# miuda-ai/lele

Measured on AMD Instinct MI355X. Metric: STFT+mel GB/s (SenseVoice front-end: PCM -> log-mel -> LFR, algorithmic bytes); SenseVoiceSmall-shaped RTF in `sensevoice`, higher is better.
Workload: dtype f32

## Files before the change

### lele_amd/csrc/frontend.hip

```cpp
#include <type_traits>
#include "common.h"
#include "fe_core.h"

#include <math.h>

#include <algorithm>

using namespace lele;

namespace {

constexpr int kMaxMelRounds = 8;

struct FeDev {
    const float* tw_re;
    const float* tw_im;
    const float2* tw;
    const float* window;
    const float* melw;
    const int* mel_start;
    const int* mel_step_off;
    int mel_rounds;
    int mel_steps;
    int n_mels;
    int lfr_m, lfr_n;
};

struct GridBlock {
    __device__ __forceinline__ unsigned x() const { return blockIdx.x; }
    __device__ __forceinline__ unsigned y() const { return blockIdx.y; }
};
struct SegBlock {
    unsigned bx;
    __device__ __forceinline__ unsigned x() const { return bx; }
    __device__ __forceinline__ unsigned y() const { return 0u; }
};

struct FeSeg {
    int64_t start, len;
    int64_t num_frames, t_lfr;
    int64_t row0;
    int64_t block0;
};

constexpr int kSumRows = 66;
constexpr int kSumPitch = 164;

__global__ __launch_bounds__(64) void fe_frame_sum_kernel(const float* __restrict__ pcm, int64_t utt_stride,
                                                          int64_t pcm_len, int64_t num_frames,
                                                          float* __restrict__ mean_out, int aligned16) {
    __shared__ __attribute__((aligned(16))) float tile[kSumRows * kSumPitch];
    const int lane = threadIdx.x;
    const int64_t f0 = (int64_t)blockIdx.x * 64;
    const float* base = pcm + (int64_t)blockIdx.y * utt_stride;
    const int64_t s0 = f0 * fe::kHop;
    constexpr int kVecPerRow = fe::kHop / 4;
    constexpr int kVecs = kSumRows * kVecPerRow;
    constexpr int kIters = (kVecs + 63) / 64;
    constexpr int kBatch = 14;
    static_assert(kIters % kBatch == 0, "batching");
    for (int b0 = 0; b0 < kIters; b0 += kBatch) {
        float4 st[kBatch];
#pragma unroll
        for (int u = 0; u < kBatch; ++u) {
            const int idx = (b0 + u) * 64 + lane;
            int64_t s = s0 + 4 * (int64_t)idx;
            if (s + 3 >= pcm_len) s = aligned16 ? ((pcm_len - 4) & ~int64_t(3)) : (pcm_len - 4);
            if (s < 0) s = 0;
            const float* src = base + s;
            if (aligned16) {
                st[u] = *reinterpret_cast<const float4*>(src);
            } else {
                st[u] = make_float4(src[0], src[1], src[2], src[3]);
            }
        }
#pragma unroll
        for (int u = 0; u < kBatch; ++u) {
            const int idx = (b0 + u) * 64 + lane;
            if (idx < kVecs) {
                float4 xv = st[u];
                xv.x *= 32768.0f;
                xv.y *= 32768.0f;
                xv.z *= 32768.0f;
                xv.w *= 32768.0f;
                const int row = idx / kVecPerRow, c = idx - row * kVecPerRow;
                *reinterpret_cast<float4*>(&tile[row * kSumPitch + 4 * c]) = xv;
            }
        }
    }
    __syncthreads();
    float sum = 0.0f;
#pragma unroll
    for (int seg = 0; seg < 3; ++seg) {
        const float* rowp = &tile[(lane + seg) * kSumPitch];
        const int nvec = seg < 2 ? kVecPerRow : (fe::kFrame - 2 * fe::kHop) / 4;
#pragma unroll 10
        for (int k = 0; k < nvec; ++k) {
            const float4 r = *reinterpret_cast<const float4*>(rowp + 4 * k);
            sum = sum + r.x;
            sum = sum + r.y;
            sum = sum + r.z;
            sum = sum + r.w;
        }
    }
    const int64_t f = f0 + lane;
    if (f < num_frames) mean_out[(int64_t)blockIdx.y * num_frames + f] = sum / (float)fe::kFrame;
}

constexpr int kFrameXchgFloats = 2 * 16 * fe::kXchgPitch;
constexpr int kWaveLdsFloats = 4 * kFrameXchgFloats;
constexpr int kPStride = 272;

struct TwLds {
    const float2* t;
    __device__ __forceinline__ float2 at(int i) const { return t[i]; }
};

template <int MODE>
__device__ __forceinline__ float lane_rot_prev(float v, int p) {
    if (MODE == 1) {
        return __builtin_bit_cast(float,
                                  __builtin_amdgcn_update_dpp(0, __builtin_bit_cast(int, v), 0x121, 0xf, 0xf, true));
    } else {
        return __shfl(v, (p + 15) & 15, 16);
    }
}

constexpr int kStdMelLen[5] = {3, 4, 6, 10, 17};
constexpr int kStdMelOff[6] = {0, 3, 7, 13, 23, 40};

template <int MODE, bool STDMEL, bool FUSED, int PASSES, bool LOWREG, class Blk>
__device__ __forceinline__ void fe_main_body(const float* __restrict__ pcm, int64_t utt_stride,
                                             int64_t num_frames, int64_t t_lfr,
                                             const float* __restrict__ means, const FeDev& tb,
                                             float* __restrict__ out, float* __restrict__ logmel_out,
                                             int aligned16, float* s_melw, Blk bl) {
    constexpr int FR = 16 * PASSES;
    constexpr int kRows = FR + 2;
    constexpr int kXFloats = FUSED ? (kRows * kSumPitch > 4 * kWaveLdsFloats ? kRows * kSumPitch : 4 * kWaveLdsFloats)
                                   : 4 * kWaveLdsFloats;
    __shared__ float2 s_tw[LOWREG ? 480 : 512];
    __shared__ __attribute__((aligned(16))) float s_x[kXFloats];
    __shared__ float s_mean[64];
    __shared__ int s_mstart[16 * (STDMEL ? 5 : kMaxMelRounds)];
    __shared__ int s_moff[kMaxMelRounds + 1];
    constexpr int kTwBase = LOWREG ? 31 : 0;

    for (int i = threadIdx.x; i < 511 - kTwBase; i += 256) s_tw[i] = tb.tw[i + kTwBase];
    if (!STDMEL)
        for (int i = threadIdx.x; i < tb.mel_steps * 16; i += 256) s_melw[i] = tb.melw[i];
    if (threadIdx.x < tb.mel_rounds * 16) s_mstart[threadIdx.x] = tb.mel_start[threadIdx.x];
    if (threadIdx.x <= tb.mel_rounds) s_moff[threadIdx.x] = tb.mel_step_off[threadIdx.x];
    const int lane = threadIdx.x & 63, wave = threadIdx.x >> 6;
    const int g = lane >> 4, p = lane & 15;
    if (FUSED) {
        const float* ubase = pcm + (int64_t)bl.y() * utt_stride;
        const int64_t s0 = (int64_t)bl.x() * FR * fe::kHop;
        constexpr int kVecPerRow = fe::kHop / 4;
        constexpr int kVecs = kRows * kVecPerRow;
        constexpr int kIters = (kVecs + 255) / 256;
        float4 st[kIters];
#pragma unroll
        for (int u = 0; u < kIters; ++u) {
            const int idx = u * 256 + (int)threadIdx.x;
            int64_t sidx = s0 + 4 * (int64_t)idx;
            if (sidx + 3 >= utt_stride) sidx = aligned16 ? ((utt_stride - 4) & ~int64_t(3)) : (utt_stride - 4);
            if (sidx < 0) sidx = 0;
            const float* src = ubase + sidx;
            if (aligned16)
                st[u] = *reinterpret_cast<const float4*>(src);
            else
                st[u] = make_float4(src[0], src[1], src[2], src[3]);
        }
#pragma unroll
        for (int u = 0; u < kIters; ++u) {
            const int idx = u * 256 + (int)threadIdx.x;
            if (idx < kVecs) {
                float4 xv = st[u];
                xv.x *= 32768.0f;
                xv.y *= 32768.0f;
                xv.z *= 32768.0f;
                xv.w *= 32768.0f;
                const int row = idx / kVecPerRow, c = idx - row * kVecPerRow;
                *reinterpret_cast<float4*>(&s_x[row * kSumPitch + 4 * c]) = xv;
            }
        }
        __syncthreads();
    }
    const int h = fe::rev4(p);
    float* xw = s_x + wave * kWaveLdsFloats;
    float* xf = xw + g * kFrameXchgFloats;
    const float* base = pcm + (int64_t)bl.y() * utt_stride;
    const float* mean_u = means + (int64_t)bl.y() * num_frames;
    const int d_out = tb.n_mels * tb.lfr_m;
    float* out_u = out ? out + (int64_t)bl.y() * t_lfr * d_out : nullptr;
    float* lm_u = logmel_out ? logmel_out + (int64_t)bl.y() * num_frames * tb.n_mels : nullptr;

    float win[fe::kQ];
    if (!LOWREG) {
#pragma unroll
        for (int q = 0; q < fe::kQ; ++q) win[q] = tb.window[p + 16 * q];
    }

    float xr[fe::kQ];
    float mean_next = 0.0f;
    auto issue_loads = [&](int pass) {
        const int64_t f = (int64_t)bl.x() * FR + wave * (4 * PASSES) + pass * 4 + g;
        const int64_t fc = f < num_frames ? f : 0;
        const float* src = base + fc * fe::kHop + p;
        if (!FUSED) mean_next = mean_u[fc];
#pragma unroll
        for (int q = 0; q < fe::kQ; ++q) xr[q] = src[16 * q];
    };
    issue_loads(0);
    if (FUSED) {
        constexpr int kVecPerRow = fe::kHop / 4;
        if (wave == 0 && lane < FR) {
            float sum = 0.0f;
#pragma unroll
            for (int seg = 0; seg < 3; ++seg) {
                const float* rowp = &s_x[(lane + seg) * kSumPitch];
                const int nvec = seg < 2 ? kVecPerRow : (fe::kFrame - 2 * fe::kHop) / 4;
#pragma unroll 10
                for (int k = 0; k < nvec; ++k) {
                    const float4 r = *reinterpret_cast<const float4*>(rowp + 4 * k);
                    sum = sum + r.x;
                    sum = sum + r.y;
                    sum = sum + r.z;
                    sum = sum + r.w;
                }
            }
            s_mean[lane] = sum / (float)fe::kFrame;
        }
    }
    __syncthreads();

    auto run_pass = [&](int pass, auto load_next_c) {
        constexpr bool load_next = decltype(load_next_c)::value;
        const int64_t f = (int64_t)bl.x() * FR + wave * (4 * PASSES) + pass * 4 + g;
        const bool valid = f < num_frames;
        const float mean = FUSED ? s_mean[wave * (4 * PASSES) + pass * 4 + g] : mean_next;
        if (LOWREG) {
            int off = 0;
            asm volatile("" : "+v"(off));
#pragma unroll
            for (int q = 0; q < fe::kQ; ++q) win[q] = tb.window[p + 16 * q + off];
        }

        float v[fe::kQ];
        const float neg_mean = -mean;
#pragma unroll
        for (int q = 0; q < fe::kQ; ++q) v[q] = __builtin_fmaf(xr[q], 32768.0f, neg_mean);
        if (load_next) issue_loads(pass + 1);
        float xin[fe::kRegs];
#pragma unroll
        for (int r = 0; r < fe::kRegs; ++r) xin[r] = 0.0f;
        float k97;
        asm("v_mov_b32 %0, 0x3f7851ec" : "=v"(k97));
#pragma unroll
        for (int q = 0; q < fe::kQ; ++q) {
            const float send = (p == 15 && q > 0) ? v[q > 0 ? q - 1 : 0] : v[q];
            const float prev = lane_rot_prev<MODE>(send, p);
            float y = fe::fsub(v[q], fe::fmul(k97, prev));
            if (q == 0) y = (p == 0) ? v[0] : y;
            xin[fe::rev5(q)] = fe::fmul(y, win[q]);
        }

        fe::cf a[fe::kRegs];
        fe::phase_a_fast(xin, a, tb.tw_re, tb.tw_im);

        float pw[2][8];
        float p256 = 0.0f;
#pragma unroll
        for (int rho = 0; rho < 2; ++rho) {
            __builtin_amdgcn_wave_barrier();
#pragma unroll
            for (int cc = 0; cc < 16; ++cc) {
                const int slot = fe::xchg_slot(h, cc);
                *reinterpret_cast<float2*>(xf + 2 * slot) = make_float2(a[rho * 16 + cc].x, a[rho * 16 + cc].y);
            }
            __builtin_amdgcn_wave_barrier();
            fe::cf bq[16];
#pragma unroll
            for (int vv = 0; vv < 16; ++vv) {
                const float2 t = *reinterpret_cast<const float2*>(xf + 2 * fe::xchg_slot(vv, p));
                bq[vv] = fe::cmk(t.x, t.y);
            }
            __builtin_amdgcn_wave_barrier();
            float re256 = 0.0f;
            fe::phase_b(bq, p, rho, [&](int i) { const float2 w = s_tw[i - kTwBase]; return fe::cmk(w.x, w.y); }, &re256);
            if (rho == 0) p256 = re256;
#pragma unroll
            for (int vv = 0; vv < 8; ++vv) {
                fe::cf z = bq[vv];
                if (vv == 0 && rho == 0) z = fe::cmk(z.x, (p == 0) ? 0.0f : z.y);
                pw[rho][vv] = fe::power(z);
            }
        }
        float* prow = xw + g * kPStride;
        __builtin_amdgcn_wave_barrier();
#pragma unroll
        for (int rho = 0; rho < 2; ++rho)
#pragma unroll
            for (int vv = 0; vv < 8; ++vv) prow[(2 * vv + rho) * 16 + p] = pw[rho][vv];
        if (p == 0) prow[256] = fe::power(p256, 0.0f);
        __builtin_amdgcn_wave_barrier();

        const int fi = (int)f, nfr = (int)num_frames, tl = (int)t_lfr;
        const int pad = (tb.lfr_m - 1) / 2;
        const int fp = fi + pad;
        const int b_first = fp % tb.lfr_n, i_first = fp / tb.lfr_n;

        float vals[STDMEL ? 5 : kMaxMelRounds];
#pragma unroll
        for (int rd = 0; rd < (STDMEL ? 5 : kMaxMelRounds); ++rd) {
            vals[rd] = 0.0f;
            if (!STDMEL && rd >= tb.mel_rounds) continue;
            const int m = rd * 16 + p;
            const int start = s_mstart[m];
            const float* pp = prow + start;
            float acc = 0.0f;
            if (STDMEL) {
                const float* wp = tb.melw + kStdMelOff[rd < 5 ? rd : 0] * 16 + p;
                float w[17];
#pragma unroll
                for (int t = 0; t < 17; ++t)
                    if (t < kStdMelLen[rd < 5 ? rd : 0]) w[t] = wp[t * 16];
#pragma unroll
                for (int t = 0; t < 17; ++t)
                    if (t < kStdMelLen[rd < 5 ? rd : 0]) acc = fe::fadd(acc, fe::fmul(w[t], pp[t]));
            } else {
                const int t0 = s_moff[rd], t1 = s_moff[rd + 1];
                const float* wp = s_melw + t0 * 16 + p;
                const int lim = 256 - start;
#pragma unroll 4
                for (int t = 0; t < t1 - t0; ++t) {
                    const float pv = pp[t < lim ? t : lim];
                    acc = fe::fadd(acc, fe::fmul(wp[t * 16], pv));
                }
            }
            {
                const float l2 = __builtin_amdgcn_logf(fmaxf(acc, 1e-5f));
                const float hi = __builtin_bit_cast(float, 0x3f317217u), lo = __builtin_bit_cast(float, 0x3377d1cfu);
                const float r = fe::fmul(l2, hi);
                vals[rd] = fe::fadd(r, fe::ffma(l2, lo, fe::ffma(l2, hi, -r)));
            }
        }
        if (valid) {
            constexpr int kR = STDMEL ? 5 : kMaxMelRounds;
            auto put = [&](float* dst) {
#pragma unroll
                for (int rd = 0; rd < kR; ++rd)
                    if (rd * 16 + p < tb.n_mels) __builtin_nontemporal_store(vals[rd], &dst[rd * 16]);
            };
            if (lm_u) put(lm_u + (int64_t)fi * tb.n_mels + p);
            if (out_u) {
                int i = i_first;
                for (int b = b_first; b < tb.lfr_m && i >= 0; b += tb.lfr_n, --i)
                    if (i < tl) put(out_u + i * d_out + b * tb.n_mels + p);
                if (fi == 0) {
                    for (int i2 = 0; i2 * tb.lfr_n - pad < 0 && i2 < tl; ++i2)
                        for (int b = 0; b < tb.lfr_m && i2 * tb.lfr_n + b - pad < 0; ++b)
                            put(out_u + i2 * d_out + b * tb.n_mels + p);
                }
                if (fi == nfr - 1) {
                    for (int i2 = tl - 1; i2 >= 0 && i2 * tb.lfr_n + (tb.lfr_m - 1) - pad > fi; --i2)
                        for (int b = tb.lfr_m - 1; b >= 0 && i2 * tb.lfr_n + b - pad > fi; --b)
                            put(out_u + i2 * d_out + b * tb.n_mels + p);
                }
            }
        }
        __builtin_amdgcn_wave_barrier();
    };
#pragma unroll 1
    for (int pass = 0; pass + 1 < PASSES; ++pass) run_pass(pass, std::true_type{});
    run_pass(PASSES - 1, std::false_type{});
}

template <int MODE, bool STDMEL, bool FUSED>
__global__ __launch_bounds__(256) void fe_main_kernel(const float* __restrict__ pcm, int64_t utt_stride, int64_t num_frames, int64_t t_lfr,
                                                      const float* __restrict__ means, FeDev tb, float* __restrict__ out,
                                                      float* __restrict__ logmel_out, int aligned16) {
    extern __shared__ float s_melw[];
    fe_main_body<MODE, STDMEL, FUSED, 4, false>(pcm, utt_stride, num_frames, t_lfr, means, tb, out, logmel_out, aligned16, s_melw,
                                                GridBlock{});
}

template <int MODE, bool STDMEL>
__global__ __launch_bounds__(256) void fe_seg_main_kernel(const float* __restrict__ pcm, const FeSeg* __restrict__ segs,
                                                          const int* __restrict__ blk_seg, FeDev tb, float* __restrict__ out) {
    extern __shared__ float s_melw[];
    const FeSeg s = segs[blk_seg[blockIdx.x]];
    const float* base = pcm + s.start;
    const int aligned16 = (((uintptr_t)base & 15) == 0) && (s.len % 4 == 0);
    fe_main_body<MODE, STDMEL, true, 4, false>(base, s.len, s.num_frames, s.t_lfr, nullptr, tb, out + s.row0 * (tb.n_mels * tb.lfr_m),
                                               nullptr, aligned16, s_melw, SegBlock{(unsigned)(blockIdx.x - s.block0)});
}
__global__ void fe_generic_mean_kernel(const float* __restrict__ pcm, int64_t rows, int64_t num_frames, int64_t pcm_len, int frame_len, int hop,
                                       float* __restrict__ mean) {
    const int64_t f = (int64_t)blockIdx.x * blockDim.x + threadIdx.x;
    if (f >= rows) return;
    const float* src = pcm + (f / num_frames) * pcm_len + (f % num_frames) * hop;
    float sum = 0.0f;
    int j = 0;
    if ((((uintptr_t)src) & 15) == 0) {
        for (; j + 16 <= frame_len; j += 16) {
            float4 v[4];
#pragma unroll
            for (int u = 0; u < 4; ++u) v[u] = *reinterpret_cast<const float4*>(src + j + 4 * u);
#pragma unroll
            for (int u = 0; u < 4; ++u) {
                sum = sum + v[u].x * 32768.0f;
                sum = sum + v[u].y * 32768.0f;
                sum = sum + v[u].z * 32768.0f;
                sum = sum + v[u].w * 32768.0f;
            }
        }
    }
    for (; j < frame_len; ++j) sum = sum + src[j] * 32768.0f;
    mean[f] = sum / (float)frame_len;
}
__global__ void fe_generic_frame_kernel(const float* __restrict__ pcm, const float* __restrict__ mean,
                                        const float* __restrict__ window, int64_t rows, int64_t num_frames, int64_t pcm_len, int frame_len, int hop,
                                        int n_fft, float* __restrict__ frames) {
    const int64_t total = rows * n_fft;
    for (int64_t i = (int64_t)blockIdx.x * blockDim.x + threadIdx.x; i < total; i += (int64_t)gridDim.x * blockDim.x) {
        const int64_t f = i / n_fft;
        const int j = (int)(i - f * n_fft);
        float v = 0.0f;
        if (j < frame_len) {
            const float* src = pcm + (f / num_frames) * pcm_len + (f % num_frames) * hop;
            const float m = mean[f];
            const float cur = fe::fsub(fe::fmul(src[j], 32768.0f), m);
            float y = cur;
            if (j >= 1) y = fe::fsub(cur, fe::fmul(0.97f, fe::fsub(fe::fmul(src[j - 1], 32768.0f), m)));
            v = fe::fmul(y, window[j]);
        }
        frames[i] = v;
    }
}
__global__ void fe_generic_mel_kernel(const float* __restrict__ power, int64_t num_frames, int n_bins, int n_mels,
                                      const int* __restrict__ mstart, const int* __restrict__ moff,
                                      const float* __restrict__ mw, float* __restrict__ logmel) {
    const int64_t total = num_frames * n_mels;
    for (int64_t i = (int64_t)blockIdx.x * blockDim.x + threadIdx.x; i < total; i += (int64_t)gridDim.x * blockDim.x) {
        const int64_t f = i / n_mels;
        const int m = (int)(i - f * n_mels);
        const float* p = power + f * n_bins + mstart[m];
        float acc = 0.0f;
        for (int t = moff[m]; t < moff[m + 1]; ++t) acc = fe::fadd(acc, fe::fmul(mw[t], p[t - moff[m]]));
        logmel[i] = __logf(fmaxf(acc, 1e-5f));
    }
}
#define FE_PAD(i) ((i) + ((i) >> 5))
__global__ __launch_bounds__(256) void fe_generic_fused_kernel(const float* __restrict__ pcm, int64_t pcm_len, int64_t num_frames, int frame_len,
                                                               int hop, int n, int log2n, int fpb, const float* __restrict__ window,
                                                               const float* __restrict__ tw_re_g, const float* __restrict__ tw_im_g, int n_mels,
                                                               const int* __restrict__ mstart, const int* __restrict__ moff,
                                                               const float* __restrict__ mw, const float* __restrict__ means,
                                                               float* __restrict__ logmel) {
    extern __shared__ float gfl[];
    const int nb = n / 2 + 1, span = (fpb - 1) * hop + frame_len;
    float* re = gfl;
    float* im = re + FE_PAD(fpb * n) + 1;
    float* pw = im + FE_PAD(fpb * n) + 1;
    float* sp = pw + fpb * nb;
    float* smean = sp + span;
    const int tid = threadIdx.x;
    const int64_t f0 = (int64_t)blockIdx.x * fpb;
    const int nfr = (int)(num_frames - f0 < fpb ? num_frames - f0 : fpb);
    const float* src = pcm + (int64_t)blockIdx.y * pcm_len + f0 * hop;
    const int have = (nfr - 1) * hop + frame_len;
    for (int i = tid; i < span; i += 256) sp[i] = i < have ? src[i] : 0.0f;
    __syncthreads();
    if (means) {
        if (tid < nfr) smean[tid] = means[(int64_t)blockIdx.y * num_frames + f0 + tid];
    } else if (tid < nfr) {
        const float* fr = sp + tid * hop;
        float sum = 0.0f;
        int j = 0;
        for (; j + 16 <= frame_len; j += 16) {
            float v[16];
#pragma unroll
            for (int u = 0; u < 16; ++u) v[u] = fr[j + u];
#pragma unroll
            for (int u = 0; u < 16; ++u) sum = sum + v[u] * 32768.0f;
        }
        for (; j < frame_len; ++j) sum = sum + fr[j] * 32768.0f;
        smean[tid] = sum / (float)frame_len;
    }
    __syncthreads();
    for (int i = tid; i < fpb * n; i += 256) {
        const int f = i >> log2n, j = i & (n - 1);
        float v = 0.0f;
        if (j < frame_len && f < nfr) {
            const float* fr = sp + f * hop;
            const float m = smean[f];
            const float cur = fe::fsub(fe::fmul(fr[j], 32768.0f), m);
            float y = cur;
            if (j >= 1) y = fe::fsub(cur, fe::fmul(0.97f, fe::fsub(fe::fmul(fr[j - 1], 32768.0f), m)));
            v = fe::fmul(y, window[j]);
        }
        const int r = (int)(__brev((unsigned)j) >> (32 - log2n));
        re[FE_PAD(f * n + r)] = v;
        im[FE_PAD(f * n + r)] = 0.0f;
    }
    __syncthreads();
    for (int s0 = 0; s0 < log2n;) {
        const int R = log2n - s0 >= 3 ? 3 : log2n - s0, h = 1 << s0, gsz = 1 << R, groups = n >> R;
        for (int idx = tid; idx < fpb * groups; idx += 256) {
            const int f = idx / groups, g = idx - f * groups;
            const int lo = g & (h - 1), base = f * n + ((g >> s0) << (s0 + R)) + lo;
            float xr[8], xi[8];
#pragma unroll
            for (int j = 0; j < 8; ++j)
                if (j < gsz) xr[j] = re[FE_PAD(base + j * h)], xi[j] = im[FE_PAD(base + j * h)];
#pragma unroll
            for (int r = 0; r < 3; ++r) {
                if (r >= R) break;
                const int half = h << r, off = half - 1;
#pragma unroll
                for (int j = 0; j < 8; ++j) {
                    if (j >= gsz || (j >> r) & 1) continue;
                    const int k = lo + (j & ((1 << r) - 1)) * h;
                    const float wr = tw_re_g[off + k], wi = tw_im_g[off + k];
                    if (half >= 4)
                        fe::bfly_fma(wr, wi, xr[j], xi[j], xr[j + (1 << r)], xi[j + (1 << r)]);
                    else
                        fe::bfly_scalar(wr, wi, xr[j], xi[j], xr[j + (1 << r)], xi[j + (1 << r)]);
                }
            }
#pragma unroll
            for (int j = 0; j < 8; ++j)
                if (j < gsz) re[FE_PAD(base + j * h)] = xr[j], im[FE_PAD(base + j * h)] = xi[j];
        }
        s0 += R;
        __syncthreads();
    }
    for (int i = tid; i < fpb * nb; i += 256) {
        const int f = i / nb, k = i - f * nb;
        const float r = re[FE_PAD(f * n + k)];
        const float q = (k == 0 || k == nb - 1) ? 0.0f : im[FE_PAD(f * n + k)];
        pw[i] = fe::power(r, q);
    }
    __syncthreads();
    for (int i = tid; i < nfr * n_mels; i += 256) {
        const int f = i / n_mels, m = i - f * n_mels;
        const float* pp = pw + f * nb + mstart[m];
        const float* wp = mw + moff[m];
        const int cnt = moff[m + 1] - moff[m];
        float acc = 0.0f;
        int t = 0;
        for (; t + 8 <= cnt; t += 8) {
            float w8[8], p8[8];
#pragma unroll
            for (int u = 0; u < 8; ++u) w8[u] = wp[t + u], p8[u] = pp[t + u];
#pragma unroll
            for (int u = 0; u < 8; ++u) acc = fe::fadd(acc, fe::fmul(w8[u], p8[u]));
        }
        for (; t < cnt; ++t) acc = fe::fadd(acc, fe::fmul(wp[t], pp[t]));
        logmel[((int64_t)blockIdx.y * num_frames + f0 + f) * n_mels + m] = __logf(fmaxf(acc, 1e-5f));
    }
}
__global__ void fe_generic_lfr_kernel(const float* __restrict__ x, int64_t t, int64_t d, int64_t m, int64_t n,
                                      int64_t t_lfr, float* __restrict__ out) {
    const int64_t d_out = d * m, total = t_lfr * d_out, pad = (m - 1) / 2;
    x += (int64_t)blockIdx.y * t * d;
    out += (int64_t)blockIdx.y * total;
    for (int64_t idx = (int64_t)blockIdx.x * blockDim.x + threadIdx.x; idx < total; idx += (int64_t)gridDim.x * blockDim.x) {
        const int64_t i = idx / d_out, rem = idx - i * d_out, block = rem / d, k = rem - block * d;
        int64_t raw = i * n + block - pad;
        raw = raw < 0 ? 0 : (raw > t - 1 ? t - 1 : raw);
        out[idx] = x[raw * d + k];
    }
}

}

struct LeleFrontend {
    LeleCtx* ctx = nullptr;
    LeleFeatureConfig cfg{};
    int64_t frame_len = 0, hop_len = 0, n_fft = 0;
    bool fast = false;
    bool std_mel = false;
    int dpp_mode = 0;
    bool fused = true;
    const float* g_window = nullptr;
    const int* g_mstart = nullptr;
    const int* g_moff = nullptr;
    const float* g_mw = nullptr;
    FeDev dev{};
    std::vector<void*> allocs;
    DevTables seg_tables;
    bool profiling = false;
    std::vector<hipEvent_t> events;
    size_t events_used = 0;
};

namespace {

static const float PI_F = 3.14159265358979323846264338327950288f;

void host_hann(int64_t size, std::vector<float>& w) {
    w.resize(size);
    if (size == 1) w[0] = 1.0f;
    for (int64_t n = 0; size > 1 && n < size; ++n) w[n] = 0.5f * (1.0f - cosf(2.0f * PI_F * (float)n / (float)(size - 1)));
}

void host_twiddles(int64_t n, std::vector<float>& re, std::vector<float>& im) {
    re.clear();
    im.clear();
    for (int64_t size = 2; size <= n; size *= 2) {
        int64_t half = size / 2, step = n / size;
        for (int64_t k = 0; k < half; ++k) {
            float angle = -2.0f * PI_F * (float)(k * step) / (float)n;
            re.push_back(cosf(angle));
            im.push_back(sinf(angle));
        }
    }
}

float hz_to_mel(float hz) { return 2595.0f * log10f(1.0f + hz / 700.0f); }
float mel_to_hz(float mel) { return 700.0f * (powf(10.0f, mel / 2595.0f) - 1.0f); }

void host_dense_mel(float sr, int64_t n_fft, int64_t n_mels, float f_min, float f_max, float* bank) {
    const int64_t n_freqs = n_fft / 2 + 1;
    const float mel_min = hz_to_mel(f_min), mel_max = hz_to_mel(f_max);
    const float mel_step = (mel_max - mel_min) / (float)(n_mels + 1);
    std::vector<float> hz(n_mels + 2), ff(n_freqs);
    for (int64_t i = 0; i < n_mels + 2; ++i) hz[i] = mel_to_hz(mel_min + (float)i * mel_step);
    for (int64_t i = 0; i < n_freqs; ++i) ff[i] = (float)i * sr / (float)n_fft;
    for (int64_t i = 0; i < n_mels; ++i) {
        const float fl = hz[i], fc = hz[i + 1], fr = hz[i + 2];
        for (int64_t j = 0; j < n_freqs; ++j) {
            const float f = ff[j];
            float val = 0.0f;
            if (f > fl && f < fc)
                val = (f - fl) / (fc - fl);
            else if (f >= fc && f < fr)
                val = (fr - f) / (fr - fc);
            bank[i * n_freqs + j] = val;
        }
    }
}

void host_sparse_mel(float sr, int64_t n_fft, int64_t n_mels, float f_min, std::vector<int>& start,
                     std::vector<std::vector<float>>& w) {
    const int64_t n_freqs = n_fft / 2 + 1;
    std::vector<float> bank((size_t)n_mels * n_freqs);
    host_dense_mel(sr, n_fft, n_mels, f_min, sr / 2.0f, bank.data());
    start.assign(n_mels, 0);
    w.assign(n_mels, {});
    for (int64_t i = 0; i < n_mels; ++i) {
        const float* row = bank.data() + i * n_freqs;
        int64_t s = 0;
        while (s < n_freqs && row[s] == 0.0f) ++s;
        int64_t e = n_freqs;
        while (e > s && row[e - 1] == 0.0f) --e;
        if (s < e) {
            start[i] = (int)s;
            w[i].assign(row + s, row + e);
        }
    }
}

template <typename T>
int upload(LeleFrontend* fe, const std::vector<T>& v, const T** out) {
    void* d = nullptr;
    size_t bytes = std::max<size_t>(v.size() * sizeof(T), 16);
    LELE_HIP_CHECK(hipMalloc(&d, bytes));
    fe->allocs.push_back(d);
    if (!v.empty()) LELE_HIP_CHECK(hipMemcpy(d, v.data(), v.size() * sizeof(T), hipMemcpyHostToDevice));
    *out = (const T*)d;
    return 0;
}

}

extern "C" {

int lele_hip_hann_window(int64_t size, float* out) {
    LELE_REQUIRE(size >= 0 && (out || size == 0), "hann_window: bad argument");
    std::vector<float> w;
    host_hann(size, w);
    if (size) memcpy(out, w.data(), (size_t)size * 4);
    return 0;
}
float lele_hip_hz_to_mel_htk(float hz) { return hz_to_mel(hz); }
float lele_hip_mel_to_hz_htk(float mel) { return mel_to_hz(mel); }
int lele_hip_mel_filterbank(float sample_rate, int64_t n_fft, int64_t n_mels, float f_min, int32_t has_f_max, float f_max, float* out) {
    LELE_REQUIRE(n_fft >= 0 && n_mels >= 0 && (out || n_mels == 0), "mel_filterbank: bad argument");
    if (n_mels) host_dense_mel(sample_rate, n_fft, n_mels, f_min, has_f_max ? f_max : sample_rate / 2.0f, out);
    return 0;
}


int lele_hip_frontend_create(LeleCtx* ctx, const LeleFeatureConfig* cfg, LeleFrontend** out) {
    LELE_REQUIRE(ctx && cfg && out, "frontend_create: NULL argument");
    LELE_REQUIRE(cfg->sample_rate > 0 && cfg->n_mels > 0 && cfg->lfr_m > 0 && cfg->lfr_n > 0,
                 "frontend_create: invalid FeatureConfig");
    LELE_HIP_CHECK(hipSetDevice(ctx->device));
    LeleFrontend* fe = new LeleFrontend();
    fe->ctx = ctx;
    fe->cfg = *cfg;
    fe->frame_len = (int64_t)((float)cfg->sample_rate * cfg->frame_length_ms / 1000.0f);
    fe->n_fft = fe->frame_len > 400 ? 1024 : 512;
    fe->hop_len = (int64_t)((float)cfg->sample_rate * cfg->frame_shift_ms / 1000.0f);
    fe->fast = (fe->frame_len == fe::kFrame && fe->hop_len == fe::kHop && fe->n_fft == fe::kNfft &&
                cfg->n_mels <= 16 * kMaxMelRounds);
    if (!fe->fast) {
        if (fe->frame_len < 1 || fe->hop_len < 1 || fe->frame_len > fe->n_fft) {
            const long long fl = (long long)fe->frame_len, hl = (long long)fe->hop_len, nf = (long long)fe->n_fft;
            delete fe;
            set_error("frontend_create: frame_len=%lld hop_len=%lld do not fit fft_len=%lld (the reference panics here)", fl, hl, nf);
            return 3;
        }
        std::vector<float> gwin;
        host_hann(fe->frame_len, gwin);
        std::vector<int> gstart;
        std::vector<std::vector<float>> gw;
        host_sparse_mel((float)cfg->sample_rate, fe->n_fft, cfg->n_mels, 20.0f, gstart, gw);
        std::vector<int> goff(cfg->n_mels + 1, 0);
        std::vector<float> gflat;
        for (int64_t m = 0; m < cfg->n_mels; ++m) {
            goff[m] = (int)gflat.size();
            gflat.insert(gflat.end(), gw[m].begin(), gw[m].end());
        }
        goff[cfg->n_mels] = (int)gflat.size();
        int rc = 0;
        rc |= upload(fe, gwin, &fe->g_window);
        rc |= upload(fe, gstart, &fe->g_mstart);
        rc |= upload(fe, goff, &fe->g_moff);
        rc |= upload(fe, gflat, &fe->g_mw);
        if (rc) {
            lele_hip_frontend_destroy(fe);
            return rc;
        }
        *out = fe;
        return 0;
    }
    std::vector<float> win, twr, twi;
    host_hann(fe->frame_len, win);
    host_twiddles(fe->n_fft, twr, twi);
    LELE_REQUIRE(twr[0] == 1.0f && twi[0] == 0.0f && twr[1] == 1.0f && twi[1] == 0.0f,
                 "frontend_create: unexpected twiddle table head");
    std::vector<float2> tw(512, make_float2(0.f, 0.f));
    for (size_t i = 0; i < twr.size(); ++i) tw[i] = make_float2(twr[i], twi[i]);
    twr.resize(512, 0.0f);
    twi.resize(512, 0.0f);
    std::vector<int> mstart;
    std::vector<std::vector<float>> mw;
    host_sparse_mel((float)cfg->sample_rate, fe->n_fft, cfg->n_mels, 20.0f, mstart, mw);
    FeDev& d = fe->dev;
    d.n_mels = (int)cfg->n_mels;
    d.lfr_m = (int)cfg->lfr_m;
    d.lfr_n = (int)cfg->lfr_n;
    d.mel_rounds = (int)((cfg->n_mels + 15) / 16);
    std::vector<int> start_pad(d.mel_rounds * 16, 0);
    std::vector<float> melw;
    std::vector<int> step_off(d.mel_rounds + 1, 0);
    int off = 0;
    for (int rd = 0; rd < d.mel_rounds; ++rd) {
        size_t maxlen = 0;
        for (int pm = 0; pm < 16; ++pm) {
            int m = rd * 16 + pm;
            if (m < cfg->n_mels) {
                start_pad[m] = mstart[m];
                maxlen = std::max(maxlen, mw[m].size());
            }
        }
        step_off[rd] = off;
        for (size_t t = 0; t < maxlen; ++t)
            for (int pm = 0; pm < 16; ++pm) {
                int m = rd * 16 + pm;
                melw.push_back((m < cfg->n_mels && t < mw[m].size()) ? mw[m][t] : 0.0f);
            }
        off += (int)maxlen;
    }
    step_off[d.mel_rounds] = off;
    d.mel_steps = off;
    fe->std_mel = (d.mel_rounds == 5 && cfg->n_mels == 80);
    for (int rd = 0; fe->std_mel && rd < 5; ++rd) {
        if (step_off[rd] != kStdMelOff[rd] || step_off[rd + 1] != kStdMelOff[rd + 1]) fe->std_mel = false;
        for (int pm = 0; pm < 16; ++pm)
            if (start_pad[rd * 16 + pm] + kStdMelLen[rd] - 1 > 256) fe->std_mel = false;
    }
    if (lab_env("LELE_HIP_FE_GENERIC_MEL")) fe->std_mel = false;
    int rc = 0;
    rc |= upload(fe, twr, &d.tw_re);
    rc |= upload(fe, twi, &d.tw_im);
    rc |= upload(fe, tw, &d.tw);
    rc |= upload(fe, win, &d.window);
    rc |= upload(fe, melw, &d.melw);
    rc |= upload(fe, start_pad, &d.mel_start);
    rc |= upload(fe, step_off, &d.mel_step_off);
    if (rc) {
        lele_hip_frontend_destroy(fe);
        return rc;
    }
    const char* env = lab_env("LELE_HIP_FE_DPP");
    fe->dpp_mode = env ? atoi(env) : 1;
    const char* envf = lab_env("LELE_HIP_FE_FUSED");
    fe->fused = envf ? atoi(envf) != 0 : true;
    *out = fe;
    return 0;
}

int lele_hip_frontend_destroy(LeleFrontend* fe) {
    if (!fe) return 0;
    (void)hipStreamSynchronize(fe->ctx->stream);
    for (void* p : fe->allocs) (void)hipFree(p);
    fe->seg_tables.release();
    for (hipEvent_t e : fe->events) (void)hipEventDestroy(e);
    delete fe;
    return 0;
}

int lele_hip_frontend_out_rows(const LeleFrontend* fe, int64_t pcm_len, int64_t* rows, int64_t* cols,
                               int64_t* num_frames) {
    LELE_REQUIRE(fe, "frontend_out_rows: fe is NULL");
    int64_t nf = 0, t = 0;
    if (pcm_len >= fe->frame_len) {
        nf = (pcm_len - fe->frame_len) / fe->hop_len + 1;
        t = (nf + fe->cfg.lfr_n - 1) / fe->cfg.lfr_n;
    }
    if (rows) *rows = t;
    if (cols) *cols = fe->cfg.n_mels * fe->cfg.lfr_m;
    if (num_frames) *num_frames = nf;
    return 0;
}

static int ilog2_i(int n) {
    int l = 0;
    while ((1 << (l + 1)) <= n) ++l;
    return l;
}
static int fe_generic(LeleFrontend* fe, const float* dpcm, int64_t batch, int64_t pcm_len, int64_t nf, int64_t t_lfr, int64_t cols,
                      float* outp, bool want_logmel, void* dmean) {
    LeleCtx* ctx = fe->ctx;
    const int64_t bins = fe->n_fft / 2 + 1, nm = fe->cfg.n_mels;
    if (fe->fused && fe->n_fft <= 4096 && fe->frame_len <= fe->n_fft && batch <= 65535) {
        const int n = (int)fe->n_fft;
        int fpb = n <= 512 ? 4 : n <= 1024 ? 2 : 1;
        if (const char* e = lab_env("LELE_HIP_FE_FPB")) fpb = std::max(1, atoi(e));
        const size_t padded = (size_t)fpb * n + (((size_t)fpb * n) >> 5) + 1;
        const size_t lds = (2 * padded + (size_t)fpb * bins + (size_t)(fpb - 1) * fe->hop_len + fe->frame_len + fpb) * 4;
        if (lds <= 96 * 1024) {
            const float *twr = nullptr, *twi = nullptr;
            LELE_TRY(fft_twiddles(ctx, n, &twr, &twi));
            LELE_HIP_CHECK(ensure_dyn_lds(reinterpret_cast<const void*>(fe_generic_fused_kernel), (int)lds));
            const int64_t per_utt_lm = nf * nm * 4;
            const int64_t ubf = want_logmel ? batch : std::max<int64_t>(1, std::min<int64_t>(batch, (int64_t(1) << 28) / std::max<int64_t>(per_utt_lm, 1)));
            void* glm = nullptr;
            if (!want_logmel) LELE_TRY(ctx->arena_alloc((size_t)ubf * nf * nm * 4, &glm));
            for (int64_t u = 0; u < batch; u += ubf) {
                const int64_t nu = std::min<int64_t>(ubf, batch - u);
                const float* up = (const float*)dpcm + u * pcm_len;
                float* lm = want_logmel ? outp + u * nf * nm : (float*)glm;
                hipLaunchKernelGGL(fe_generic_mean_kernel, dim3((unsigned)((nu * nf + 63) / 64)), dim3(64), 0, ctx->stream, up, nu * nf, nf, pcm_len,
                                   (int)fe->frame_len, (int)fe->hop_len, (float*)dmean);
                hipLaunchKernelGGL(fe_generic_fused_kernel, dim3((unsigned)((nf + fpb - 1) / fpb), (unsigned)nu), dim3(256), lds, ctx->stream, up,
                                   pcm_len, nf, (int)fe->frame_len, (int)fe->hop_len, n, ilog2_i(n), fpb, fe->g_window, twr, twi, (int)nm,
                                   fe->g_mstart, fe->g_moff, fe->g_mw, (const float*)dmean, lm);
                if (!want_logmel) {
                    dim3 lg((unsigned)std::max<int64_t>(1, std::min<int64_t>((t_lfr * cols + 255) / 256, 8192)), (unsigned)nu);
                    hipLaunchKernelGGL(fe_generic_lfr_kernel, lg, dim3(256), 0, ctx->stream, (const float*)lm, nf, nm, fe->cfg.lfr_m,
                                       fe->cfg.lfr_n, t_lfr, outp + u * t_lfr * cols);
                }
            }
            LELE_HIP_CHECK(hipGetLastError());
            return 0;
        }
    }
    const int64_t per_utt = nf * (4 + fe->n_fft * 4 + bins * 4 + nm * 4);
    const int64_t ub = std::max<int64_t>(1, std::min<int64_t>(std::min<int64_t>(batch, 65535), (int64_t(1) << 28) / std::max<int64_t>(per_utt, 1)));
    void *gm = nullptr, *gf = nullptr, *gp = nullptr, *gl = nullptr;
    LELE_TRY(ctx->arena_alloc((size_t)ub * nf * 4, &gm));
    LELE_TRY(ctx->arena_alloc((size_t)ub * nf * fe->n_fft * 4, &gf));
    LELE_TRY(ctx->arena_alloc((size_t)ub * nf * bins * 4, &gp));
    if (!want_logmel) LELE_TRY(ctx->arena_alloc((size_t)ub * nf * nm * 4, &gl));
    auto blocks = [](int64_t n) { return dim3((unsigned)std::max<int64_t>(1, std::min<int64_t>((n + 255) / 256, 8192))); };
    for (int64_t u = 0; u < batch; u += ub) {
        const int64_t nu = std::min<int64_t>(ub, batch - u), rows = nu * nf;
        const float* up = (const float*)dpcm + u * pcm_len;
        float* lm = want_logmel ? outp + u * nf * nm : (float*)gl;
        hipLaunchKernelGGL(fe_generic_mean_kernel, dim3((unsigned)((rows + 63) / 64)), dim3(64), 0, ctx->stream, up, rows, nf, pcm_len,
                           (int)fe->frame_len, (int)fe->hop_len, (float*)gm);
        hipLaunchKernelGGL(fe_generic_frame_kernel, blocks(rows * fe->n_fft), dim3(256), 0, ctx->stream, up, (const float*)gm,
                           fe->g_window, rows, nf, pcm_len, (int)fe->frame_len, (int)fe->hop_len, (int)fe->n_fft, (float*)gf);
        LELE_TRY(fft_rows_power(ctx, (const float*)gf, rows, fe->n_fft, (float*)gp));
        hipLaunchKernelGGL(fe_generic_mel_kernel, blocks(rows * nm), dim3(256), 0, ctx->stream, (const float*)gp, rows, (int)bins,
                           (int)nm, fe->g_mstart, fe->g_moff, fe->g_mw, lm);
        if (!want_logmel) {
            dim3 lg = blocks(t_lfr * cols);
            lg.y = (unsigned)nu;
            hipLaunchKernelGGL(fe_generic_lfr_kernel, lg, dim3(256), 0, ctx->stream, (const float*)lm, nf, nm,
                               fe->cfg.lfr_m, fe->cfg.lfr_n, t_lfr, outp + u * t_lfr * cols);
        }
    }
    LELE_HIP_CHECK(hipGetLastError());
    return 0;
}

static int fe_run(LeleFrontend* fe, const LeleTensor* pcm, int64_t batch, int64_t pcm_len, LeleBuf* out,
                  bool want_logmel, int64_t* out_shape, int32_t* out_rank) {
    LeleCtx* ctx = fe->ctx;
    LELE_HIP_CHECK(hipSetDevice(ctx->device));
    LELE_REQUIRE(pcm->dtype == LELE_F32, "frontend: pcm must be f32");
    int64_t t_lfr = 0, cols = 0, nf = 0;
    lele_hip_frontend_out_rows(fe, pcm_len, &t_lfr, &cols, &nf);
    if (nf == 0 || batch == 0) {
        out->bytes = 0;
        if (out_rank) *out_rank = 0;
        return 0;
    }
    LELE_TRY(ctx->arena_reset());
    const void* dpcm = nullptr;
    LELE_TRY(ctx->dev_ptr(pcm, &dpcm));
    void* dmean = nullptr;
    LELE_TRY(ctx->get_scratch((size_t)batch * nf * sizeof(float), &dmean));
    const size_t out_elems = want_logmel ? (size_t)batch * nf * fe->cfg.n_mels : (size_t)batch * t_lfr * cols;
    LELE_TRY(out->reserve(out_elems * sizeof(float)));
    if (!fe->fast) {
        LELE_TRY(fe_generic(fe, (const float*)dpcm, batch, pcm_len, nf, t_lfr, cols, (float*)out->data, want_logmel, dmean));
        if (want_logmel) {
            if (batch == 1) return set_shape(out_shape, out_rank, {nf, fe->cfg.n_mels});
            return set_shape(out_shape, out_rank, {batch, nf, fe->cfg.n_mels});
        }
        return 0;
    }
    const int aligned16 = ((uintptr_t)dpcm % 16 == 0) && (pcm_len % 4 == 0);
    dim3 grid((unsigned)((nf + 63) / 64), (unsigned)batch);
    hipEvent_t* ev = nullptr;
    if (fe->profiling) {
        if (fe->events_used + 3 > fe->events.size()) {
            for (int i = 0; i < 3; ++i) {
                hipEvent_t e;
                LELE_HIP_CHECK(hipEventCreate(&e));
                fe->events.push_back(e);
            }
        }
        ev = &fe->events[fe->events_used];
        fe->events_used += 3;
        LELE_HIP_CHECK(hipEventRecord(ev[0], ctx->stream));
    }
    if (!fe->fused)
        hipLaunchKernelGGL(fe_frame_sum_kernel, grid, dim3(64), 0, ctx->stream, (const float*)dpcm, pcm_len, pcm_len, nf,
                           (float*)dmean, aligned16);
    if (ev) LELE_HIP_CHECK(hipEventRecord(ev[1], ctx->stream));
    const size_t mel_lds = (size_t)fe->dev.mel_steps * 16 * sizeof(float);
    float* o = want_logmel ? nullptr : (float*)out->data;
    float* lm = want_logmel ? (float*)out->data : nullptr;
#define FE_LAUNCH(MODE, STD, FUS)                                                                                     \
    hipLaunchKernelGGL((fe_main_kernel<MODE, STD, FUS>), grid, dim3(256), mel_lds, ctx->stream, (const float*)dpcm, \
                       pcm_len, nf, t_lfr, (const float*)dmean, fe->dev, o, lm, aligned16)
#define FE_LAUNCH2(MODE, STD) \
    do {                      \
        if (fe->fused)        \
            FE_LAUNCH(MODE, STD, true); \
        else                  \
            FE_LAUNCH(MODE, STD, false); \
    } while (0)
    if (fe->dpp_mode == 1) {
        if (fe->std_mel) FE_LAUNCH2(1, true); else FE_LAUNCH2(1, false);
    } else {
        if (fe->std_mel) FE_LAUNCH2(0, true); else FE_LAUNCH2(0, false);
    }
#undef FE_LAUNCH2
#undef FE_LAUNCH
    LELE_HIP_CHECK(hipGetLastError());
    if (ev) LELE_HIP_CHECK(hipEventRecord(ev[2], ctx->stream));
    if (want_logmel) {
        if (batch == 1) return set_shape(out_shape, out_rank, {nf, fe->cfg.n_mels});
        return set_shape(out_shape, out_rank, {batch, nf, fe->cfg.n_mels});
    }
    return 0;
}

int lele_hip_frontend_compute(LeleFrontend* fe, const LeleTensor* pcm, LeleBuf* out, int64_t* out_shape,
                              int32_t* out_rank) {
    LELE_REQUIRE(fe && pcm && out, "frontend_compute: NULL argument");
    const int64_t n = numel(pcm);
    LELE_TRY(fe_run(fe, pcm, 1, n, out, false, out_shape, out_rank));
    if (out->bytes == 0) return 0;
    int64_t t = 0, cols = 0;
    lele_hip_frontend_out_rows(fe, n, &t, &cols, nullptr);
    return set_shape(out_shape, out_rank, {t, cols});
}

int lele_hip_frontend_compute_batch(LeleFrontend* fe, const LeleTensor* pcm, LeleBuf* out, int64_t* out_shape,
                                    int32_t* out_rank) {
    LELE_REQUIRE(fe && pcm && out, "frontend_compute_batch: NULL argument");
    LELE_REQUIRE(pcm->rank == 2, "frontend_compute_batch: pcm must be [batch, pcm_len]");
    const int64_t batch = pcm->shape[0], n = pcm->shape[1];
    LELE_TRY(fe_run(fe, pcm, batch, n, out, false, out_shape, out_rank));
    if (out->bytes == 0) return 0;
    int64_t t = 0, cols = 0;
    lele_hip_frontend_out_rows(fe, n, &t, &cols, nullptr);
    return set_shape(out_shape, out_rank, {batch, t, cols});
}

int lele_hip_frontend_logmel(LeleFrontend* fe, const LeleTensor* pcm, LeleBuf* out, int64_t* out_shape,
                             int32_t* out_rank) {
    LELE_REQUIRE(fe && pcm && out, "frontend_logmel: NULL argument");
    if (pcm->rank == 2) return fe_run(fe, pcm, pcm->shape[0], pcm->shape[1], out, true, out_shape, out_rank);
    return fe_run(fe, pcm, 1, numel(pcm), out, true, out_shape, out_rank);
}

struct SegLayout {
    const LeleFrontend* fe;
    const int64_t* starts;
    const int64_t* lengths;
    int64_t count;
    const int64_t* rows;
};
static void build_seg_table(const void* arg, std::vector<char>& blob) {
    const SegLayout& L = *(const SegLayout*)arg;
    std::vector<FeSeg> segs;
    std::vector<int> blk;
    for (int64_t i = 0; i < L.count; ++i) {
        int64_t t = 0, nf = 0;
        lele_hip_frontend_out_rows(L.fe, L.lengths[i], &t, nullptr, &nf);
        if (nf == 0) continue;
        const int64_t nb = (nf + 63) / 64;
        segs.push_back(FeSeg{L.starts[i], L.lengths[i], nf, t, L.rows[i], (int64_t)blk.size()});
        blk.insert(blk.end(), (size_t)nb, (int)segs.size() - 1);
    }
    blob.resize(segs.size() * sizeof(FeSeg) + blk.size() * sizeof(int));
    memcpy(blob.data(), segs.data(), segs.size() * sizeof(FeSeg));
    memcpy(blob.data() + segs.size() * sizeof(FeSeg), blk.data(), blk.size() * sizeof(int));
}

int lele_hip_frontend_compute_segments(LeleFrontend* fe, const LeleTensor* pcm, const int64_t* starts, const int64_t* lengths, int64_t count,
                                       LeleBuf* out, int64_t* row_offsets, int64_t* out_shape, int32_t* out_rank) {
    LELE_REQUIRE(fe && pcm && out && row_offsets, "frontend_compute_segments: NULL argument");
    LELE_REQUIRE(count >= 0 && (count == 0 || (starts && lengths)), "frontend_compute_segments: bad segment arrays (count %lld)",
                 (long long)count);
    LELE_REQUIRE(pcm->dtype == LELE_F32 && pcm->rank == 1, "frontend_compute_segments: pcm must be f32 [N]");
    const int64_t n = pcm->shape[0];
    for (int64_t i = 0; i < count; ++i)
        LELE_REQUIRE(starts[i] >= 0 && lengths[i] >= 0 && starts[i] <= n - lengths[i],
                     "frontend_compute_segments: segment %lld (start %lld, length %lld) lies outside the %lld samples of pcm", (long long)i,
                     (long long)starts[i], (long long)lengths[i], (long long)n);
    int64_t cols = fe->cfg.n_mels * fe->cfg.lfr_m, blocks = 0, max_nf = 0;
    row_offsets[0] = 0;
    for (int64_t i = 0; i < count; ++i) {
        int64_t t = 0, nf = 0;
        lele_hip_frontend_out_rows(fe, lengths[i], &t, nullptr, &nf);
        row_offsets[i + 1] = row_offsets[i] + t;
        blocks += (nf + 63) / 64;
        max_nf = std::max(max_nf, nf);
    }
    const int64_t rows = row_offsets[count];
    if (rows == 0) {
        out->bytes = 0;
        if (out_rank) *out_rank = 0;
        return 0;
    }
    LELE_REQUIRE(blocks < (int64_t(1) << 31), "frontend_compute_segments: %lld blocks exceed the grid", (long long)blocks);
    LeleCtx* ctx = fe->ctx;
    LELE_HIP_CHECK(hipSetDevice(ctx->device));
    LELE_TRY(ctx->arena_reset());
    const void* dpcm = nullptr;
    LELE_TRY(ctx->dev_ptr(pcm, &dpcm));
    LELE_TRY(out->reserve((size_t)rows * cols * sizeof(float)));
    float* o = (float*)out->data;
    if (!fe->fast) {
        void* dmean = nullptr;
        LELE_TRY(ctx->get_scratch((size_t)max_nf * sizeof(float), &dmean));
        const size_t mark = ctx->arena_used;
        for (int64_t i = 0; i < count; ++i) {
            int64_t t = 0, nf = 0;
            lele_hip_frontend_out_rows(fe, lengths[i], &t, nullptr, &nf);
            if (nf == 0) continue;
            LELE_TRY(fe_generic(fe, (const float*)dpcm + starts[i], 1, lengths[i], nf, t, cols, o + row_offsets[i] * cols, false, dmean));
            ctx->arena_used = mark;
        }
        return set_shape(out_shape, out_rank, {rows, cols});
    }
    std::string key((size_t)count * 16, '\0');
    memcpy(&key[0], starts, (size_t)count * 8);
    memcpy(&key[(size_t)count * 8], lengths, (size_t)count * 8);
    const SegLayout lay{fe, starts, lengths, count, row_offsets};
    const void* table = nullptr;
    LELE_TRY(fe->seg_tables.get(ctx, std::move(key), build_seg_table, &lay, &table));
    int64_t nseg = 0;
    for (int64_t i = 0; i < count; ++i) nseg += lengths[i] >= fe->frame_len;
    const FeSeg* dsegs = (const FeSeg*)table;
    const int* dblk = (const int*)(dsegs + nseg);
    const size_t mel_lds = (size_t)fe->dev.mel_steps * 16 * sizeof(float);
#define FE_SEG_LAUNCH(MODE, STD)                                                                                                 \
    hipLaunchKernelGGL((fe_seg_main_kernel<MODE, STD>), dim3((unsigned)blocks), dim3(256), mel_lds, ctx->stream, (const float*)dpcm, \
                       dsegs, dblk, fe->dev, o)
    if (fe->dpp_mode == 1) {
        if (fe->std_mel) FE_SEG_LAUNCH(1, true); else FE_SEG_LAUNCH(1, false);
    } else {
        if (fe->std_mel) FE_SEG_LAUNCH(0, true); else FE_SEG_LAUNCH(0, false);
    }
#undef FE_SEG_LAUNCH
    LELE_HIP_CHECK(hipGetLastError());
    return set_shape(out_shape, out_rank, {rows, cols});
}

int lele_hip_frontend_set_profiling(LeleFrontend* fe, int on) {
    LELE_REQUIRE(fe, "frontend_set_profiling: fe is NULL");
    fe->profiling = on != 0;
    fe->events_used = 0;
    return 0;
}

int lele_hip_frontend_profile_read(LeleFrontend* fe, float* sum_kernel_ms, float* main_kernel_ms, int64_t* runs) {
    LELE_REQUIRE(fe, "frontend_profile_read: fe is NULL");
    LELE_HIP_CHECK(hipStreamSynchronize(fe->ctx->stream));
    double a = 0, b = 0;
    const size_t n = fe->events_used / 3;
    for (size_t i = 0; i < n; ++i) {
        float m0 = 0, m1 = 0;
        LELE_HIP_CHECK(hipEventElapsedTime(&m0, fe->events[3 * i], fe->events[3 * i + 1]));
        LELE_HIP_CHECK(hipEventElapsedTime(&m1, fe->events[3 * i + 1], fe->events[3 * i + 2]));
        a += m0;
        b += m1;
    }
    if (sum_kernel_ms) *sum_kernel_ms = n ? (float)(a / n) : 0.f;
    if (main_kernel_ms) *main_kernel_ms = n ? (float)(b / n) : 0.f;
    if (runs) *runs = (int64_t)n;
    fe->events_used = 0;
    return 0;
}

}
```

Measured before the change: 1784.

## Stage PCM tile and twiddles into LDS via global_load_lds DMA

In the fused frontend kernel, the PCM tile is now copied straight from global memory into the padded LDS layout with global_load_lds 16-byte DMA, and the twiddle table is loaded the same way by one wave. This replaces the register round trip and the scale-by-32768 on store. The scaling moves into the mean computation via FMA, and the raw samples are already rescaled per lane in the main pass. Twiddle table pointers are also forced into the constant address space as scalar-loaded values. The change adds an env toggle and relies on a magic division trick and a manual waitcnt. It risks correctness at tile edges and in how the pre-scaled LDS values are consumed later.

```diff
diff --git a/lele_amd/csrc/frontend.hip b/lele_amd/csrc/frontend.hip
--- a/lele_amd/csrc/frontend.hip
+++ b/lele_amd/csrc/frontend.hip
@@ -24,6 +24,7 @@
     int mel_steps;
     int n_mels;
     int lfr_m, lfr_n;
+    int tile_dma;
 };
 
 struct GridBlock {
@@ -115,6 +116,16 @@
     const float2* t;
     __device__ __forceinline__ float2 at(int i) const { return t[i]; }
 };
+
+__device__ __forceinline__ void fe_dma16(const void* gsrc, __attribute__((address_space(3))) char* lds_dst) {
+    __builtin_amdgcn_global_load_lds((const __attribute__((address_space(1))) void*)gsrc, lds_dst, 16, 0, 0);
+}
+
+__device__ __forceinline__ const float* fe_const_table(const float* t, int pass) {
+    auto c = (const __attribute__((address_space(4))) float*)t;
+    asm("" : "+s"(c) : "s"(pass));
+    return (const float*)c;
+}
 
 template <int MODE>
 __device__ __forceinline__ float lane_rot_prev(float v, int p) {
@@ -146,45 +157,73 @@
     __shared__ int s_moff[kMaxMelRounds + 1];
     constexpr int kTwBase = LOWREG ? 31 : 0;
 
-    for (int i = threadIdx.x; i < 511 - kTwBase; i += 256) s_tw[i] = tb.tw[i + kTwBase];
+    const int lane = threadIdx.x & 63, wave = threadIdx.x >> 6;
+    const int g = lane >> 4, p = lane & 15;
+    constexpr int kVecPerRow = fe::kHop / 4;
+    constexpr int kVecs = kRows * kVecPerRow;
+    constexpr int kIters = (kVecs + 255) / 256;
+    constexpr bool kTwDma = FUSED && !LOWREG;
+    const bool tile_dma = FUSED && !LOWREG && aligned16 && tb.tile_dma;
+    float4 st[FUSED ? kIters : 1];
+    if constexpr (FUSED) {
+        const float* run = pcm + (int64_t)bl.y() * utt_stride + (int64_t)bl.x() * FR * fe::kHop;
+        const int64_t rem64 = utt_stride - (int64_t)bl.x() * FR * fe::kHop;
+        const int rem = (int)(rem64 < (1 << 20) ? rem64 : (1 << 20));
+        if (tile_dma) {
+            constexpr int kSlotsPerRow = kSumPitch / 4;
+            constexpr int kDma = (FR - 1 + 2) * kSlotsPerRow + (fe::kFrame - 2 * fe::kHop) / 4;
+            constexpr int kDmaInstr = (kDma + 63) / 64;
+            static_assert(kDmaInstr * 64 * 4 <= kXFloats, "the tile DMA stays inside s_x");
+            auto* tile_lds = (__attribute__((address_space(3))) char*)s_x;
+            static_assert(kSlotsPerRow == 41 && kDmaInstr * 64 * 1599 < (1 << 24), "i / 41 == (i * 1599) >> 16 for every slot");
+            const unsigned last = 4u * (unsigned)rem - 16u;
+            const int wave_s = __builtin_amdgcn_readfirstlane(wave);
+#pragma unroll
+            for (int u = 0; 4 * u < kDmaInstr; ++u) {
+                const unsigned i = 256u * u + threadIdx.x;
+                const unsigned ob = 16u * (i - ((i * 1599u) >> 16));
+                if (4 * u + 3 < kDmaInstr || 4 * u + wave_s < kDmaInstr)
+                    fe_dma16(reinterpret_cast<const char*>(run) + (ob < last ? ob : last), tile_lds + (4 * u + wave_s) * 1024);
+            }
+        }
+        if (kTwDma && wave == 3) {
+            auto* tw_lds = (__attribute__((address_space(3))) char*)s_tw;
+#pragma unroll
+            for (int k = 0; k < 4; ++k)
+                fe_dma16(reinterpret_cast<const char*>(tb.tw) + 1024 * k + 16 * lane, tw_lds + 1024 * k);
+        }
+        if (!tile_dma) {
+#pragma unroll
+            for (int u = 0; u < kIters; ++u) {
+                const int idx = u * 256 + (int)threadIdx.x;
+                int o = 4 * idx;
+                if (o + 3 >= rem) o = aligned16 ? ((rem - 4) & ~3) : (rem - 4);
+                const float* src = run + o;
+                if (aligned16)
+                    st[u] = *reinterpret_cast<const float4*>(src);
+                else
+                    st[u] = make_float4(src[0], src[1], src[2], src[3]);
+            }
+        }
+    }
+    if (!kTwDma)
+        for (int i = threadIdx.x; i < 511 - kTwBase; i += 256) s_tw[i] = tb.tw[i + kTwBase];
     if (!STDMEL)
         for (int i = threadIdx.x; i < tb.mel_steps * 16; i += 256) s_melw[i] = tb.melw[i];
     if (threadIdx.x < tb.mel_rounds * 16) s_mstart[threadIdx.x] = tb.mel_start[threadIdx.x];
     if (threadIdx.x <= tb.mel_rounds) s_moff[threadIdx.x] = tb.mel_step_off[threadIdx.x];
-    const int lane = threadIdx.x & 63, wave = threadIdx.x >> 6;
-    const int g = lane >> 4, p = lane & 15;
     if (FUSED) {
-        const float* ubase = pcm + (int64_t)bl.y() * utt_stride;
-        const int64_t s0 = (int64_t)bl.x() * FR * fe::kHop;
-        constexpr int kVecPerRow = fe::kHop / 4;
-        constexpr int kVecs = kRows * kVecPerRow;
-        constexpr int kIters = (kVecs + 255) / 256;
-        float4 st[kIters];
-#pragma unroll
-        for (int u = 0; u < kIters; ++u) {
-            const int idx = u * 256 + (int)threadIdx.x;
-            int64_t sidx = s0 + 4 * (int64_t)idx;
-            if (sidx + 3 >= utt_stride) sidx = aligned16 ? ((utt_stride - 4) & ~int64_t(3)) : (utt_stride - 4);
-            if (sidx < 0) sidx = 0;
-            const float* src = ubase + sidx;
-            if (aligned16)
-                st[u] = *reinterpret_cast<const float4*>(src);
-            else
-                st[u] = make_float4(src[0], src[1], src[2], src[3]);
-        }
-#pragma unroll
-        for (int u = 0; u < kIters; ++u) {
-            const int idx = u * 256 + (int)threadIdx.x;
-            if (idx < kVecs) {
-                float4 xv = st[u];
-                xv.x *= 32768.0f;
-                xv.y *= 32768.0f;
-                xv.z *= 32768.0f;
-                xv.w *= 32768.0f;
-                const int row = idx / kVecPerRow, c = idx - row * kVecPerRow;
-                *reinterpret_cast<float4*>(&s_x[row * kSumPitch + 4 * c]) = xv;
-            }
-        }
+        if (!tile_dma) {
+#pragma unroll
+            for (int u = 0; u < kIters; ++u) {
+                const int idx = u * 256 + (int)threadIdx.x;
+                if (idx < kVecs) {
+                    const int row = idx / kVecPerRow, c = idx - row * kVecPerRow;
+                    *reinterpret_cast<float4*>(&s_x[row * kSumPitch + 4 * c]) = st[u];
+                }
+            }
+        }
+        __builtin_amdgcn_s_waitcnt(0x0F70);
         __syncthreads();
     }
     const int h = fe::rev4(p);
@@ -214,7 +253,6 @@
     };
     issue_loads(0);
     if (FUSED) {
-        constexpr int kVecPerRow = fe::kHop / 4;
         if (wave == 0 && lane < FR) {
             float sum = 0.0f;
 #pragma unroll
@@ -224,10 +262,10 @@
 #pragma unroll 10
                 for (int k = 0; k < nvec; ++k) {
                     const float4 r = *reinterpret_cast<const float4*>(rowp + 4 * k);
-                    sum = sum + r.x;
-                    sum = sum + r.y;
-                    sum = sum + r.z;
-                    sum = sum + r.w;
+                    sum = __builtin_fmaf(r.x, 32768.0f, sum);
+                    sum = __builtin_fmaf(r.y, 32768.0f, sum);
+                    sum = __builtin_fmaf(r.z, 32768.0f, sum);
+                    sum = __builtin_fmaf(r.w, 32768.0f, sum);
                 }
             }
             s_mean[lane] = sum / (float)fe::kFrame;
@@ -267,7 +305,7 @@
         }
 
         fe::cf a[fe::kRegs];
-        fe::phase_a_fast(xin, a, tb.tw_re, tb.tw_im);
+        fe::phase_a_fast(xin, a, fe_const_table(tb.tw_re, pass), fe_const_table(tb.tw_im, pass));
 
         float pw[2][8];
         float p256 = 0.0f;
@@ -802,6 +840,8 @@
     fe->dpp_mode = env ? atoi(env) : 1;
     const char* envf = lab_env("LELE_HIP_FE_FUSED");
     fe->fused = envf ? atoi(envf) != 0 : true;
+    const char* envd = getenv("LELE_HIP_FE_TILE_DMA");
+    d.tile_dma = envd && *envd ? atoi(envd) != 0 : 1;
     *out = fe;
     return 0;
 }
```

Result: faster. 1845 (median of 6 runs) (+3.4%).
